# cunkai/index-tts-ipex

Hardware: AMD Instinct MI355X
Metric: audio_sec_per_sec (higher is better)
Workload: dtype bf16; 1 GPU; IndexTTS-1.5, 1 utterance(s)/GPU x 2 sentences x (L=105 text tokens, T=480 mel codes), prompt 511 frames, greedy fixed-length decode, rep_penalty 10; utterances_per_gpu=1, decode_batch=2

## Files before the change

### index-tts-ipex_amd/csrc/decode_engine.hip

```cpp
#include <cstdlib>
#include <type_traits>

#include "itts_decode.h"
#include "itts_engine_kernel.h"
#include "itts_sampler_dev.h"
#include "decode_pinned.h"

#ifndef ITTS_KV_PREFETCH
#define ITTS_KV_PREFETCH 1
#endif
#ifndef ITTS_EARLY_KV
#define ITTS_EARLY_KV 0
#endif

namespace itts {
namespace {

typedef unsigned int u32x4 __attribute__((ext_vector_type(4)));
typedef float f32x4 __attribute__((ext_vector_type(4)));
typedef uint32_t u32x2 __attribute__((ext_vector_type(2)));
typedef bf16_t bf16x2_t __attribute__((ext_vector_type(2)));
typedef unsigned long long u64;

template <int CTRL>
// ... 393 lines not shown
      for (int e = 0; e < 4; ++e) r2.xv[j][e] = ln_affine_rn(r2.xv[j][e], gm[j][e], bt[j][e]);
    ln_row_moments<K>(r2, 0.f, red + RED2 + grp2 * 8, tr);
  }
  __syncthreads();
  if (grp >= 0) {
    ln_row_norm<K>(r, 0.f, red + RED2 + grp * 8, eps);
    ln_row_store<K>(r, sxb + grp * (K / 2), tr);
  }
  if (NB > 4 && grp2 >= 0) {
    ln_row_norm<K>(r2, 0.f, red + RED2 + grp2 * 8, eps);
    ln_row_store<K>(r2, sxb + grp2 * (K / 2), tr);
  }
  __syncthreads();
}

template <int NB, bool ANC>
__global__ __launch_bounds__(1024) void decode_engine_kernel(EngArgs a) {
  constexpr int D = ENG_D, H = ENG_H, DH = 64, NCU = ENG_NCU;
  constexpr int GPH = NCU / H;
  constexpr int QO = 3 * DH / GPH;
  constexpr int HO = D / NCU;
  constexpr int FO = 4 * D / NCU;
  constexpr int NCW = 11;
  static_assert(GPH * QO == 3 * DH && HO * NCU == D && FO * NCU == 4 * D && (FO % 2) == 0, "partition");
  static_assert(QO <= 2 * NCW && HO <= NCW && FO / 2 <= NCW, "wave assignment");
  constexpr int NIT = 3, NSPLIT = 4, SLOTS = 32, LPK = 8, VEC = 8, UNC = 2;
  constexpr int SD = 2;
  static_assert(ATTN_NSPLIT == NSPLIT, "split count of the launch path");
  static_assert(NB <= ENG_MAX_ROWS, "LDS budget");

  extern __shared__ __attribute__((aligned(1024))) unsigned char smem[];
// ... 26 lines not shown
  const unsigned lds0 = (unsigned)(uintptr_t)(__attribute__((address_space(3))) unsigned char*)smem;
  const unsigned S0 = lds0, S1 = lds0 + SLOT, S2 = SLOT3 ? lds0 + 2 * SLOT : S1;
  static_assert(SLOT + SLOTB + (SLOT3 ? SLOTC : 0) + NB * D * 2 + NB * 4 * D * 2 + (SLOT3 ? NB * D * 4 + NB * D * 2 : 0) + (NB > 4 ? 512 : 256) +
                        (NB > 4 ? NB : 4) * 32 + (3 * DH + 16 * DH + 32 + NSPLIT * DH + 8 + 1) * 4 <= 160 * 1024, "LDS budget");
  const unsigned own_lds = lds0 + (unsigned)(reinterpret_cast<unsigned char*>(own) - smem);

  const int t = threadIdx.x, lane = t & 63;
  const int wave = __builtin_amdgcn_readfirstlane(t >> 6);
  const int cu = blockIdx.x;
  const bool gw = wave < 4;
  const bool lw = wave == 4;
  const bool cwv = wave > 4;
  const int cw = wave - 5;
  const int gh = cu / GPH, gm = cu % GPH;
  const bool qcu = cu < H * GPH;
  const bool acu = qcu && gm < NB;
  const int an0 = (gm / 4) * D + gh * DH + (gm % 4) * QO;

  Rt rt;
  rt.t0 = __builtin_amdgcn_s_memrealtime();
  const u64 clk0 = __builtin_amdgcn_s_memtime();
  rt.limit = a.timeout_ticks;
  rt.ctr = a.ctr;
  rt.dead = false;
  rt.first_delay = a.first_delay;
  rt.pass_sleep = a.pass_sleep;
  rt.tag = __builtin_amdgcn_readfirstlane(a.ctr[0]);
  const int prefix = __builtin_amdgcn_readfirstlane(a.prefix[0]);
  const int my_pos = acu ? __builtin_amdgcn_readfirstlane(prefix + a.len[acu ? gm : 0]) : 0;
  const int my_ks = acu ? __builtin_amdgcn_readfirstlane(a.kv_start[acu ? gm : 0]) : 0;
  const int my_par = (ANC && acu) ? __builtin_amdgcn_readfirstlane(a.len[acu ? gm : 0] & 1) : 0;

  if (t == 0) *own = 0;
  unsigned phase = 0;
  auto phase_done = [&](int ln_) {
    if (cwv && ln_ == 0) __hip_atomic_fetch_add(own, 1u, __ATOMIC_RELAXED, __HIP_MEMORY_SCOPE_WORKGROUP);
    ++phase;
  };
  if (lw) {
    if (SLOT3) dma_rows<HO, D>(a.L[0].wp, a.L[0].bp, cu * HO, S2, lane);
    if (qcu && HALFB) {
      dma_rows_at<QA1, D>(a.L[0].wa, an0, S0 + QOFF1, lane);
      dma_rows_at<QO - QA1, D>(a.L[0].wa, an0 + QA1, S0 + 256, lane);
      if (lane < QO) dma4(a.L[0].ba + an0 + lane, S0);
    } else if (qcu) {
      dma_rows<QO, D>(a.L[0].wa, a.L[0].ba, an0, S0, lane);
    }
  }
  if (t < NB * HO) hown[(t / HO) * 8 + t % HO] = a.h[(size_t)(t / HO) * D + cu * HO + t % HO];

  __builtin_amdgcn_s_waitcnt(0x0F70);
  constexpr size_t LSTRIDE = (size_t)NB * D * 15 / 2;
  constexpr size_t OQKV = 0, OCTX = (size_t)NB * 3 * D, OH1 = OCTX + NB * D / 2, OACT = OH1 + NB * D, OH2 = OACT + NB * 2 * D;
  for (int l = 0; l < a.NL; ++l) {
    const EngLayerW& w = a.L[l];
    int tl = t;
    asm volatile("" : "+v"(tl));
    const int ll = tl & 63;
    u64* __restrict__ G = a.gran + (size_t)l * LSTRIDE;

    constexpr int NIT_ = 3, NSPLIT_ = 4, SLOTS_ = 32, LPK_ = 8, VEC_ = 8, UNC_ = 2;
    KVec kr[2 * NIT_], vr[2 * NIT_];
    const int a_sp = wave >> 2, a_atid = (wave & 3) * 64 + ll, a_slot = a_atid / LPK_, a_sub = a_atid % LPK_;
    const size_t a_lo = ((size_t)l * a.B * H + (size_t)(acu ? gm : 0) * H + gh) * a.Smax * DH;
    const uint8_t* a_arow = nullptr;
    size_t a_lbase = 0;
    if constexpr (ANC) {
      a_arow = a.anc + ((size_t)my_par * a.B + (acu ? gm : 0)) * a.Smax;
      a_lbase = ((size_t)l * a.B + (size_t)((acu ? gm : 0) / a.nb) * a.nb) * H;
    }
    auto krow = [&](int j) -> const bf16_t* {
      if constexpr (ANC) return a.kc + ((a_lbase + (size_t)min((int)a_arow[j], a.nb - 1) * H + gh) * a.Smax + j) * DH;
      return a.kc + a_lo + (size_t)j * DH;
    };
    auto vrow = [&](int j) -> const bf16_t* {
      if constexpr (ANC) return a.vc + ((a_lbase + (size_t)min((int)a_arow[j], a.nb - 1) * H + gh) * a.Smax + j) * DH;
      return a.vc + a_lo + (size_t)j * DH;
    };
    auto kv_issue = [&](auto lo_c, auto hi_c) {
      constexpr int LO = decltype(lo_c)::value, HI = decltype(hi_c)::value;
#pragma unroll
      for (int u = LO; u < HI; ++u)
        if (u < UNC_ || (u * NSPLIT_ + a_sp) * SLOTS_ < my_pos + 1) {
          const int j = min((u * NSPLIT_ + a_sp) * SLOTS_ + a_slot, a.Smax - 1);
          kr[u].load(krow(j) + a_sub * VEC_);
          vr[u].load(vrow(j) + a_sub * VEC_);
        }
      __builtin_amdgcn_sched_barrier(0);
    };
    constexpr int EKV = ITTS_EARLY_KV;
    using Ic0 = std::integral_constant<int, 0>;
    using IcE = std::integral_constant<int, EKV>;
    using IcN = std::integral_constant<int, 2 * NIT_>;
    unsigned pf_sink = 0;
    if (ITTS_KV_PREFETCH && acu && cwv) {
      const int c0 = cw * 64 + ll;
      for (int j = my_ks + c0; j < my_pos; j += NCW * 64) {
        const char* pk = reinterpret_cast<const char*>(krow(j));
        const char* pv = reinterpret_cast<const char*>(vrow(j));
        asm volatile("global_load_dword %0, %1, off\n\tglobal_load_dword %0, %1, off offset:64\n\t"
                     "global_load_dword %0, %2, off\n\tglobal_load_dword %0, %2, off offset:64"
                     : "+v"(pf_sink)
                     : "v"(pk), "v"(pv)
                     : "memory");
      }
    }
    const bool early_kv = acu && EKV > 0;
    if (early_kv && cwv) kv_issue(Ic0{}, IcE{});

    if (gw) {
      if (l == 0) {
        for (int i = tl; i < NB * D; i += 256) xf[i] = a.h[i];
        __builtin_amdgcn_s_waitcnt(0x0F70);
      } else {
        wait_own(own_lds, NCW * phase, rt);
        sweep2<(NB * D / 2 + 255) / 256, false>(G - LSTRIDE + OH2, NB * D / 2 / a.fake_div, tl, rt, [&](int i, uint32_t v) { xf[i] = __uint_as_float(v); }, rt.first_delay);
      }
      if (early_kv) kv_issue(Ic0{}, IcE{});
    } else if (lw) {
      if (HALFB && l > 0 && qcu) {
        wait_own(own_lds, NCW * phase, rt);
        dma_rows_at<QO - QA1, D>(w.wa, an0 + QA1, S0 + 256, ll);
      }
      dma_wait_keep<0>();
      if (early_kv) kv_issue(Ic0{}, IcE{});
    }
    ENG_STAMP(0)
    __syncthreads();
    ENG_STAMP(1)
    ln_to_sxb<NB, D>(xf, xn, red, tl, a.eps);
    if (SLOT3) {
      if (lw && !acu) dma_rows<HO, 4 * D>(w.w2, w.b2, cu * HO, S1, ll);
    } else if (lw) {
      dma_rows<HO, D>(w.wp, w.bp, cu * HO, S1, ll);
    }
    if (qcu && cwv) {
#pragma unroll
      for (int s = 0; s < 2; ++s) {
        const int r = cw + NCW * s;
        if (r < QO) {
// ... 4 lines not shown
          float mine = 0.f;
#pragma unroll
          for (int b = 0; b < NB; ++b) {
            const float x = wave_sum_rl(acc[b]);
            mine = ll == b ? x : mine;
          }
          if (ll < NB) {
            st_gran(G + OQKV + (size_t)ll * 3 * D + an0 + r, rt.tag, __float_as_uint(mine + reinterpret_cast<const float*>(W0)[r]));
            if (a.dbg && l == a.dbg_layer) a.dbg[(size_t)ll * 3 * D + an0 + r] = mine + reinterpret_cast<const float*>(W0)[r];
          }
        }
      }
    }

    phase_done(ll);
    if (a.early_fc > 0 && lw && !acu) {
      wait_own(own_lds, NCW * phase, rt);
      for (int z = 0; z < a.early_fc; ++z) __builtin_amdgcn_s_sleep(1);
      dma_rows<FO, D>(w.wf, w.bf, cu * FO, S0, ll);
    }
    ENG_STAMP(8)

    if (acu) {
      const int sp = a_sp, atid = a_atid, slot = a_slot, sub = a_sub;
      bf16_t* kb = a.kc + a_lo;
      bf16_t* vb = a.vc + a_lo;
      kv_issue(IcE{}, IcN{});
      const int pos = my_pos, S = pos + 1, ks = my_ks;
      __builtin_amdgcn_sched_barrier(0);
      if (gw && tl < 3 * DH) {
        const u64* __restrict__ p = G + OQKV + (size_t)gm * 3 * D + (tl / DH) * D + gh * DH + tl % DH;
        wait_own(own_lds, NCW * phase, rt);
        unsigned spins = 0;
        while (!rt.dead) {
          const u64 x = ld_gran1(p);
          if ((unsigned)(x >> 32) == rt.tag) {
            qkvs[tl] = __uint_as_float((uint32_t)x);
            break;
          }
          if (spin_fail(rt, spins)) break;
          __builtin_amdgcn_s_sleep(1);
        }
      }
      ENG_STAMP(2)
      if (ITTS_KV_PREFETCH && cwv) asm volatile("s_waitcnt vmcnt(0)" : "+v"(pf_sink) : : "memory");
      __syncthreads();
      float qr[VEC];
      const bool own = atid < LPK && sp == 0;
#pragma unroll
      for (int i = 0; i < VEC; ++i) qr[i] = qkvs[sub * VEC + i] * a.scale;
      if (own) {
#pragma unroll
        for (int i = 0; i < VEC; ++i) {
          kb[(size_t)pos * DH + sub * VEC + i] = (bf16_t)qkvs[DH + sub * VEC + i];
          vb[(size_t)pos * DH + sub * VEC + i] = (bf16_t)qkvs[2 * DH + sub * VEC + i];
        }
      }
      float m = -INFINITY, lsum = 0.f, acc[VEC];
#pragma unroll
      for (int i = 0; i < VEC; ++i) acc[i] = 0.f;
      auto score = [&](const KVec& kk) {
        float sc = 0.f;
#pragma unroll
        for (int i = 0; i < VEC; ++i) sc = fmaf(qr[i], kk.get(i), sc);
        sc = dpp_add<0xB1>(sc);
        sc = dpp_add<0x4E>(sc);
        sc = dpp_add<0x141>(sc);
        return sc;
      };
      {
        float sc[2 * NIT + 1];
#pragma unroll
        for (int u = 0; u < 2 * NIT; ++u) {
          const int j = (u * NSPLIT + sp) * SLOTS + slot;
          sc[u] = -INFINITY;
          if (u < UNC || (u * NSPLIT + sp) * SLOTS < S) {
            const float tt = score(kr[u]);
            sc[u] = (j < S && j >= ks && j != pos) ? tt : -INFINITY;
          }
        }
        {
          float tt = 0.f;
#pragma unroll
          for (int i = 0; i < VEC; ++i) tt = fmaf(qr[i], own ? (float)(bf16_t)qkvs[DH + sub * VEC + i] : 0.f, tt);
          tt = dpp_add<0xB1>(tt);
          tt = dpp_add<0x4E>(tt);
          tt = dpp_add<0x141>(tt);
          sc[2 * NIT] = (slot == 0 && sp == 0) ? tt : -INFINITY;
        }
        float mw = sc[0];
#pragma unroll
        for (int u = 1; u <= 2 * NIT; ++u) mw = fmaxf(mw, sc[u]);
        if (mw > -INFINITY) {
#pragma unroll
          for (int u = 0; u < 2 * NIT; ++u)
            if (u < UNC || (u * NSPLIT + sp) * SLOTS < S) {
              const float p = __expf(sc[u] - mw);
              lsum += p;
#pragma unroll
              for (int i = 0; i < VEC; ++i) acc[i] = fmaf(p, vr[u].get(i), acc[i]);
            }
          const float p = __expf(sc[2 * NIT] - mw);
          lsum += p;
#pragma unroll
          for (int i = 0; i < VEC; ++i) acc[i] = fmaf(p, own ? (float)(bf16_t)qkvs[2 * DH + sub * VEC + i] : 0.f, acc[i]);
          m = mw;
        }
      }
      auto consume = [&](const KVec& kk, const KVec& vv, int j) {
        const bool ok = j < S && j >= ks && j != pos;
        float sc = score(kk);
        sc = ok ? sc : -INFINITY;
        const float mn = fmaxf(m, sc);
        const float corr = mn > -INFINITY ? __expf(m - mn) : 1.f;
        const float p = ok ? __expf(sc - mn) : 0.f;
        lsum = fmaf(lsum, corr, p);
#pragma unroll
        for (int i = 0; i < VEC; ++i) acc[i] = fmaf(p, ok ? vv.get(i) : 0.f, acc[i] * corr);
        m = mn;
      };
      for (int cb = 2 * NIT; (cb * NSPLIT + sp) * SLOTS < S; cb += SD) {
        KVec k2[SD], v2[SD];
#pragma unroll
        for (int u = 0; u < SD; ++u) {
          const int j = min(((cb + u) * NSPLIT + sp) * SLOTS + slot, a.Smax - 1);
          k2[u].load(krow(j) + sub * VEC);
          v2[u].load(vrow(j) + sub * VEC);
        }
#pragma unroll
        for (int u = 0; u < SD; ++u) consume(k2[u], v2[u], ((cb + u) * NSPLIT + sp) * SLOTS + slot);
      }
      auto bfly_max = [&](float x, int o) {
        if (o == 8) return fmaxf(x, __int_as_float(__builtin_amdgcn_update_dpp(0, __float_as_int(x), 0x128, 0xf, 0xf, true)));
        const u32x2 r = o == 16 ? __builtin_amdgcn_permlane16_swap(__float_as_uint(x), __float_as_uint(x), false, false)
                                : __builtin_amdgcn_permlane32_swap(__float_as_uint(x), __float_as_uint(x), false, false);
        return fmaxf(__uint_as_float(r[0]), __uint_as_float(r[1]));
      };
      auto bfly_sum = [&](float x, int o) {
        if (o == 8) return x + __int_as_float(__builtin_amdgcn_update_dpp(0, __float_as_int(x), 0x128, 0xf, 0xf, true));
        const u32x2 r = o == 16 ? __builtin_amdgcn_permlane16_swap(__float_as_uint(x), __float_as_uint(x), false, false)
                                : __builtin_amdgcn_permlane32_swap(__float_as_uint(x), __float_as_uint(x), false, false);
        return __uint_as_float(r[0]) + __uint_as_float(r[1]);
      };
      float M = m;
#pragma unroll
      for (int o = LPK; o < 64; o <<= 1) M = bfly_max(M, o);
      const float sc0 = M > -INFINITY ? __expf(m - M) : 0.f;
      lsum *= sc0;
#pragma unroll
      for (int i = 0; i < VEC; ++i) acc[i] *= sc0;
#pragma unroll
      for (int o = LPK; o < 64; o <<= 1) {
        lsum = bfly_sum(lsum, o);
#pragma unroll
        for (int i = 0; i < VEC; ++i) acc[i] = bfly_sum(acc[i], o);
      }
      if (ll < LPK)
#pragma unroll
        for (int i = 0; i < VEC; ++i) so[wave * DH + ll * VEC + i] = acc[i];
      if (ll == 0) {
        smx[wave] = M;
        slx[wave] = lsum;
      }
      __syncthreads();
      if (atid < DH) {
        float MM = smx[4 * sp];
#pragma unroll
        for (int i = 1; i < 4; ++i) MM = fmaxf(MM, smx[4 * sp + i]);
        float o = 0.f, L = 0.f;
#pragma unroll
        for (int i = 0; i < 4; ++i) {
          const float e = smx[4 * sp + i] > -INFINITY ? __expf(smx[4 * sp + i] - MM) : 0.f;
          o = fmaf(e, so[(4 * sp + i) * DH + atid], o);
          L = fmaf(e, slx[4 * sp + i], L);
        }
        po[sp * DH + atid] = o;
        if (atid == 0) {
          pml[sp] = MM;
          pml[NSPLIT + sp] = L;
        }
      }
      __syncthreads();
      if (tl < DH / 2) {
        const float Mx = fmaxf(fmaxf(pml[0], pml[1]), fmaxf(pml[2], pml[3]));
        float wgt[NSPLIT], L = 0.f;
#pragma unroll
        for (int s2 = 0; s2 < NSPLIT; ++s2) {
          wgt[s2] = pml[s2] > -INFINITY ? __expf(pml[s2] - Mx) : 0.f;
          L = fmaf(wgt[s2], pml[NSPLIT + s2], L);
        }
        const float inv = 1.f / L;
        float xm[2];
#pragma unroll
        for (int e = 0; e < 2; ++e) {
          float v = 0.f;
#pragma unroll
          for (int s2 = 0; s2 < NSPLIT; ++s2) v = fmaf(wgt[s2], po[s2 * DH + 2 * tl + e], v);
          xm[e] = v * inv;
        }
        st_gran(G + OCTX + (size_t)gm * (D / 2) + gh * (DH / 2) + tl, rt.tag, pack_bf16(xm[0], xm[1]));
      }
      ENG_STAMP(3)
    }

    if (gw) {
      if (acu)
        sweep2<(NB * D / 4 + 255) / 256, false>(G + OCTX, NB * D / 4, tl, rt, [&](int i, uint32_t v) { xc[i] = v; }, rt.first_delay);
      else
        sweep2<(NB * D / 4 + 255) / 256, true>(G + OCTX, NB * D / 4, tl, rt, [&](int i, uint32_t v) { xc[i] = v; }, a.ctx_delay);
    } else if (!SLOT3 && lw) {
      dma_wait_keep<0>();
    }
    ENG_STAMP(4)
    __syncthreads();
    if (lw && !(a.early_fc > 0 && !acu)) {
      if (a.thin_fc)
        dma_rows<FO, D, 12>(w.wf, w.bf, cu * FO, S0, ll);
      else
        dma_rows<FO, D>(w.wf, w.bf, cu * FO, S0, ll);
    }
    if (cwv && cw < HO) {
      float acc[NB];
#pragma unroll
      for (int b = 0; b < NB; ++b) acc[b] = 0.f;
      dots<NB, D>(W2 + 256 + cw * D * 2, xc, ll, acc);
      float mine = 0.f;
#pragma unroll
      for (int b = 0; b < NB; ++b) {
        const float x = wave_sum_rl(acc[b]);
        mine = ll == b ? x : mine;
// ... 288 lines not shown
    }
  }
  if (cu == 0 && t == 0) a.ctr[0] = rt.tag + 1 == 0 ? 1u : rt.tag + 1;
  if (a.stamp && t == 0) {
    const u64 c1 = __builtin_amdgcn_s_memtime(), r1 = __builtin_amdgcn_s_memrealtime();
    a.stamp[(size_t)cu * a.NL * 16 + 15] = (unsigned)((c1 - clk0) * 1000 / (r1 - rt.t0 + 1));
    if (a.NL >= 3) {
      a.stamp[((size_t)cu * a.NL + 1) * 16 + 15] = (unsigned)rt.t0;
      a.stamp[((size_t)cu * a.NL + 2) * 16 + 15] = (unsigned)r1;
    }
  }
}

}

size_t eng_gran_count(int layers) { return (size_t)layers * ENG_MAX_ROWS * ENG_D * 15 / 2 + ENG_CAND_WORDS; }

int decode_engine_layers(const EngArgs& a, hipStream_t s) {
  ITTS_REQUIRE(a.B >= 1 && a.B <= ENG_MAX_ROWS && a.NL >= 1 && a.NL <= ENG_MAX_LAYERS && a.gran && a.h && a.kc && a.vc && a.ctr, "decode_engine: bad arguments");
  const size_t lds = 160 * 1024;
#define ITTS_ENG_GO(NB, ANC_)                                                                                                   \
  {                                                                                                                             \
    static bool attr = false;                                                                                                   \
    if (!attr) {                                                                                                                \
      ITTS_HIP_CHECK(hipFuncSetAttribute(reinterpret_cast<const void*>(&decode_engine_kernel<NB, ANC_>),                        \
                                         hipFuncAttributeMaxDynamicSharedMemorySize, (int)lds));                                \
      attr = true;                                                                                                              \
    }                                                                                                                           \
    hipLaunchKernelGGL((decode_engine_kernel<NB, ANC_>), dim3(ENG_NCU), dim3(1024), lds, s, a);                                 \
  }
  if (a.anc) {
    ITTS_REQUIRE(a.nb >= 2 && a.nb <= a.B && a.B % a.nb == 0, "decode_engine: beam ancestry needs B to be a multiple of 2 <= nb <= B");
    if (a.B == 2) ITTS_ENG_GO(2, true)
    else if (a.B == 3) ITTS_ENG_GO(3, true)
    else if (a.B == 4) ITTS_ENG_GO(4, true)
    else if (a.B == 5) ITTS_ENG_GO(5, true)
    else ITTS_ENG_GO(6, true)
  } else if (a.B == 1) ITTS_ENG_GO(1, false)
  else if (a.B == 2) ITTS_ENG_GO(2, false)
  else if (a.B == 3) ITTS_ENG_GO(3, false)
  else if (a.B == 4) ITTS_ENG_GO(4, false)
  else if (a.B == 5) ITTS_ENG_GO(5, false)
  else ITTS_ENG_GO(6, false)
#undef ITTS_ENG_GO
  ITTS_HIP_CHECK(hipGetLastError());
  return OK;
}

}
```

### index-tts-ipex_amd/csrc/engine.h

```cpp
#pragma once
#include <map>
#include <utility>
#include <string>
#include <unordered_map>
#include <vector>

#include "../../include/itts_hip.h"
#include "itts_decode.h"
#include "itts_engine_kernel.h"
#include "itts_kernels.h"

namespace itts {

struct Tensor {
  const void* p = nullptr;
  int dt = 0, nd = 0;
  int64_t d[4] = {0, 0, 0, 0};
  int64_t numel() const {
    int64_t n = 1;
    for (int i = 0; i < nd; ++i) n *= d[i];
    return n;
  }
};

// ... 115 lines not shown
  int *cand_tok = nullptr, *cand_n = nullptr;
  int *hyp_tok = nullptr, *hyp_len = nullptr, *hyp_order = nullptr, *hyp_n = nullptr, *hyp_counter = nullptr, *beam_done = nullptr;
  float *hyp_score = nullptr, *hyp_worst = nullptr;
  size_t beam_cap = 0;
  int beam_rows = 0, beam_gen = 0, beam_smax = 0;
  unsigned long long* gran = nullptr;
  int* fuse_err = nullptr;
  int fuse_failed = 0;
  int fuse = 0, graph_fuse = 0;
  unsigned long long* eng_gran = nullptr;
  unsigned* eng_ctr = nullptr;
  int eng_off = 0;
  int eng_force = 0;
  int eng_failed = 0;
  int graph_eng = 0;
  int graph_mode = 0;
  float typical_mass = 0.f, graph_typical = 0.f;
  float* scores2 = nullptr;
  int* forced = nullptr;
  int use_forced = 0, graph_forced = 0;
  int host_sample = 0, graph_host_sample = 0;
  int input_n = 0, graph_input_n = 0;
  int last_mode = 0;
  float graph_penalty = 0.f;
  bool active = false;
};

struct Engine {
  itts_config cfg;
  int adt = 0;
// ... 81 lines not shown
  std::vector<int32_t> forced_host;
  int forced_B = 0, forced_n = 0;
  int gpt_status(int* steps, int* n_unf, hipStream_t s);
  int gpt_fetch(int32_t* codes, float* logits, hipStream_t s);
  int gpt_latent(const float* cond, const int32_t* text_ids, int L, const int32_t* codes, int T, void* latent_out,
                 hipStream_t s);
  int gpt_latent_batch(const float* cond, const int32_t* text_ids, const int* Ls, const int32_t* codes, const int* Ts,
                       int nseq, void* latent_out, hipStream_t s);
  int bigvgan(const void* latent, const float* spk, int B, int T, float* wav, hipStream_t s);
  int dvae_decode(const int32_t* codes, int B, int T, void* mel_out, hipStream_t s);
  int dvae_encode(const void* mel, int B, int T, int32_t* codes_host, hipStream_t s);

  int gpt_layers_full(float* h, int B, int S, const int* kv_start_dev, bool write_cache, hipStream_t s);
  int decode_step_launch(hipStream_t s);
  bool engine_usable() const;
  int ensure_engine_state(hipStream_t s);
  int engine_check(hipStream_t s);
  int head_and_sample(hipStream_t s, bool have_logits = false, bool sampled = false);
  int sample_from_logits(hipStream_t s, bool sampled = false);
  SamplerArgs greedy_sampler_args(const float* lg_in, bool typical) const;
  int ensure_decode_state(int B, int Smax, int max_gen, hipStream_t s);
  template <typename F>
  int two_pass(F&& body, hipStream_t s) {
    dry = true;
    ws_reset();
    int st = body();
    dry = false;
    if (st != OK) return st;
    ITTS_TRY(ws_reserve(ws_off + 4096, s));
    ws_reset();
// ... 6 lines not shown
```

### index-tts-ipex_amd/csrc/itts_engine_kernel.h

```cpp
#pragma once
#include "itts_common.h"
#include "itts_decode.h"

namespace itts {

constexpr int ENG_D = 1280, ENG_H = 20, ENG_NCU = 256, ENG_MAX_ROWS = 6;
constexpr int ENG_MAX_LAYERS = 24;
constexpr bool ENG_DEFAULT_ON = true;

struct EngLayerW {
  const bf16_t *wa, *wp, *wf, *w2;
  const float *ba, *bp, *bf, *b2;
};

struct EngArgs {
  EngLayerW L[ENG_MAX_LAYERS];
  unsigned long long* gran = nullptr;
  float* h = nullptr;
  bf16_t* kc = nullptr;
  bf16_t* vc = nullptr;
  const int* len = nullptr;
  const int* kv_start = nullptr;
  const int* prefix = nullptr;
  unsigned* ctr = nullptr;
// ... 2 lines not shown
  int NL = 0, B = 0, Smax = 0;
  float scale = 0.125f, eps = 1e-5f;
  unsigned timeout_ticks = 2000000;
  int first_delay = 14, pass_sleep = 1;
  int ctx_delay = 0, act_delay = 16;
  const bf16_t* head_w = nullptr;
  const float* head_b = nullptr;
  const float* lnf_g = nullptr;
  const float* lnf_b = nullptr;
  float* logits = nullptr;
  int V = 0;
  int fold_sampler = 0;
  SamplerArgs samp;
  unsigned long long* cand = nullptr;
  int early_fc = 0;
  int early_kv = 1;
  int fake_div = 1;
  int thin_fc = 0;
  float* dbg = nullptr;
  int dbg_layer = -1;
  unsigned* stamp = nullptr;
};

size_t eng_gran_count(int layers);
constexpr size_t ENG_CAND_WORDS = (size_t)ENG_MAX_ROWS * ENG_NCU * 2;
int decode_engine_layers(const EngArgs& a, hipStream_t s);

}
```

### index-tts-ipex_amd/csrc/model_gpt.hip

```cpp
#include <algorithm>
#include <atomic>
#include <cstdio>
#include <cmath>
#include <cstring>
#include <mutex>

#include <cstdlib>

#include "engine.h"

namespace itts {

namespace {

struct RowDesc {
  int kind, a, b, pad;
};

template <typename TW>
__global__ void gpt_embed_rows_kernel(float* __restrict__ h, const RowDesc* __restrict__ rd, const float* __restrict__ cond,
                                      const TW* __restrict__ text_emb, const TW* __restrict__ text_pos,
                                      const TW* __restrict__ mel_emb, const TW* __restrict__ mel_pos, int D) {
  const int r = blockIdx.x;
  const RowDesc d = rd[r];
// ... 132 lines not shown
  if (hipGetDevice(&dev) != hipSuccess) return false;
  int ncu = ncu_of[dev & 63].load(std::memory_order_relaxed);
  if (ncu == 0) {
    if (hipDeviceGetAttribute(&ncu, hipDeviceAttributeMultiprocessorCount, dev) != hipSuccess || ncu <= 0) ncu = -1;
    ncu_of[dev & 63].store(ncu, std::memory_order_relaxed);
  }
  const itts_config& c = cfg;
  if ((env_off && !ds.eng_force) || ds.eng_off || ds.eng_failed || ncu != ENG_NCU) return false;
  if (ds.fuse && !ds.fuse_failed) return false;
  if (adt != BF16 || ds.B < 1 || ds.B > ENG_MAX_ROWS || ds.nb < 1 || ds.B % ds.nb != 0 || (ds.nb > 1 && !ds.anc)) return false;
  if (c.model_dim != ENG_D || c.heads != ENG_H || c.layers < 1 || c.layers > ENG_MAX_LAYERS || ds.Smax > 2048 || ds.Smax % 256 != 0) return false;
  for (const GptLayerW& L : gpt.layers)
    for (const Lin* l : {&L.attn, &L.proj, &L.fc, &L.proj2})
      if (l->dt != BF16 || l->w8 || !l->b || l->taps != 1) return false;
  return true;
}

int Engine::ensure_engine_state(hipStream_t s) {
  DecodeState& d = ds;
  if (d.eng_gran) return OK;
  const itts_config& c = cfg;
  for (int l = 0; l < c.layers; ++l) {
    const GptLayerW& L = gpt.layers[l];
    ITTS_REQUIRE(L.attn.N == 3 * ENG_D && L.attn.Cin == ENG_D && L.proj.N == ENG_D && L.proj.Cin == ENG_D &&
                     L.fc.N == 4 * ENG_D && L.fc.Cin == ENG_D && L.proj2.N == ENG_D && L.proj2.Cin == 4 * ENG_D,
                 "decode engine: projection shapes");
  }
  const size_t gb = eng_gran_count(c.layers) * 8;
  ITTS_TRY(dev_alloc((void**)&d.eng_gran, gb));
  ITTS_TRY(dev_alloc((void**)&d.eng_ctr, 64));
// ... 527 lines not shown
    ea.scale = 1.f / std::sqrt((float)dh);
    static const int e_tap = getenv("ITTS_TAP_LAYER") ? atoi(getenv("ITTS_TAP_LAYER")) : -1;
    if (debug && e_tap >= 0 && e_tap < eng_first && !dry) {
      ea.dbg = ds.act;
      ea.dbg_layer = e_tap;
    }
    static const int e_fd_env = getenv("ITTS_ENGINE_FIRST_DELAY") ? atoi(getenv("ITTS_ENGINE_FIRST_DELAY")) : -1;
    static const int e_ad_env = getenv("ITTS_ENGINE_ACT_DELAY") ? atoi(getenv("ITTS_ENGINE_ACT_DELAY")) : -1;
    const int e_fd = e_fd_env >= 0 ? e_fd_env : (B <= 2 ? 14 : 12);
    const int e_ad = e_ad_env >= 0 ? e_ad_env : (B <= 2 ? 16 : B <= 4 ? 8 : 4);
    static const int e_ps = getenv("ITTS_ENGINE_PASS_SLEEP") ? atoi(getenv("ITTS_ENGINE_PASS_SLEEP")) : 1;
    static const int e_thin = getenv("ITTS_ENGINE_THIN_FC") ? atoi(getenv("ITTS_ENGINE_THIN_FC")) : 0;
    ea.thin_fc = e_thin;
    static const int e_early = getenv("ITTS_ENGINE_EARLY_FC") ? atoi(getenv("ITTS_ENGINE_EARLY_FC")) : -1;
    ea.early_fc = e_early >= 0 ? e_early : 74;
    ea.first_delay = e_fd;
    static const int e_fake = getenv("ITTS_ENG_FAKE_DIV") ? atoi(getenv("ITTS_ENG_FAKE_DIV")) : 1;
    ea.fake_div = e_fake < 1 ? 1 : e_fake;
    static const int e_ekv = getenv("ITTS_ENGINE_EARLY_KV") ? atoi(getenv("ITTS_ENGINE_EARLY_KV")) : 1;
    ea.early_kv = e_ekv;
    static const int e_cd = getenv("ITTS_ENGINE_CTX_DELAY") ? atoi(getenv("ITTS_ENGINE_CTX_DELAY")) : 0;
    ea.ctx_delay = e_cd;
    ea.act_delay = e_ad;
    ea.pass_sleep = e_ps;
    if (const char* tt = getenv("ITTS_ENGINE_TIMEOUT_TICKS")) ea.timeout_ticks = (unsigned)atol(tt);
    static const bool e_stamps = getenv("ITTS_ENGINE_STAMPS") != nullptr;
    if (debug && e_stamps && !dry) ea.stamp = (unsigned*)ds.scores2;
    ds.last_mode = eng_first > 0;
    static const bool e_head = !(getenv("ITTS_ENGINE_HEAD") && atoi(getenv("ITTS_ENGINE_HEAD")) == 0);
    const bool fold_head = e_head && eng_first == c.layers && gpt.head.dt == BF16 && !gpt.head.w8 && gpt.head.b && gpt.head.Cin == ENG_D &&
// ... 337 lines not shown
  ITTS_HIP_CHECK(hipGetDevice(&dev));
  EngineGate& g = engine_gate(dev);
  std::lock_guard<std::mutex> lk(g.mu);
  if (!g.ev) ITTS_HIP_CHECK(hipEventCreateWithFlags(&g.ev, hipEventDisableTiming));
  else ITTS_HIP_CHECK(hipStreamWaitEvent(s, g.ev, 0));
  const int rc = gpt_decode_steps(nsteps, s);
  ITTS_HIP_CHECK(hipEventRecord(g.ev, s));
  return rc;
}

int Engine::gpt_decode_steps(int nsteps, hipStream_t s) {
  ITTS_REQUIRE(nsteps >= 0, "gpt_decode: nsteps < 0");
  if (use_graph && s != nullptr) {
    DecodeState& d = ds;
    const bool stale = !d.graph || d.graph_B != d.B || d.graph_Smax != d.Smax || d.graph_max_gen != d.max_gen ||
                       d.graph_forced != d.use_forced || d.graph_input_n != d.input_n || d.graph_host_sample != d.host_sample || d.graph_fuse != (d.fuse && !d.fuse_failed) || d.graph_eng != (int)engine_usable() || d.graph_nb != d.nb || d.graph_beam_sample != d.beam_sample ||
                       d.graph_length_penalty != d.length_penalty || d.graph_typical != d.typical_mass || d.graph_penalty != d.penalty || d.graph_suppress != d.suppress_stop || d.graph_sample != d.do_sample ||
                       d.graph_top_k != d.top_k || d.graph_top_p != d.top_p || d.graph_temperature != d.temperature;
    static const int GK = [] {
      const char* e = getenv("ITTS_GRAPH_STEPS");
      const int v = e ? atoi(e) : 8;
      return v < 1 ? 1 : (v > 32 ? 32 : v);
    }();
    if (stale && nsteps > 0) {
      for (hipGraphExec_t* ge : {&d.graph, &d.graphK})
        if (*ge) {
          (void)hipGraphExecDestroy(*ge);
          *ge = nullptr;
        }
      for (int which = 0; which < (GK > 1 ? 2 : 1); ++which) {
        hipGraph_t g = nullptr;
// ... 5 lines not shown
          if (g) (void)hipGraphDestroy(g);
          return st;
        }
        ITTS_HIP_CHECK(ee);
        ITTS_HIP_CHECK(hipGraphInstantiate(which ? &d.graphK : &d.graph, g, nullptr, nullptr, 0));
        (void)hipGraphDestroy(g);
      }
      d.graph_B = d.B;
      d.graph_Smax = d.Smax;
      d.graph_max_gen = d.max_gen;
      d.graph_forced = d.use_forced;
      d.graph_input_n = d.input_n;
      d.graph_host_sample = d.host_sample;
      d.graph_fuse = d.fuse && !d.fuse_failed;
      d.graph_eng = (int)engine_usable();
      d.graph_mode = d.last_mode;
      d.graph_nb = d.nb;
      d.graph_beam_sample = d.beam_sample;
      d.graph_length_penalty = d.length_penalty;
      d.graph_typical = d.typical_mass;
      d.graph_penalty = d.penalty;
      d.graph_suppress = d.suppress_stop;
      d.graph_sample = d.do_sample;
      d.graph_top_k = d.top_k;
      d.graph_top_p = d.top_p;
      d.graph_temperature = d.temperature;
    }
    d.last_mode = d.graph_mode;
    int left = nsteps;
    if (d.graphK)
// ... 160 lines not shown
```

Measured before the change: 179.5 audio-s/s.

## Spread per-row decode attention splits across four workgroups with global partial merge

For small decode batches (up to 3 rows), each row's attention over the KV cache is split across four workgroups of the head group instead of four wave groups within one workgroup. The non-zero splits write partial max/sum/output to a new global partials region and the split-0 workgroup merges them. This spreads KV-cache reads across more CUs and adjusts the prefetch and early-FC scheduling to match. The cost is an extra cross-workgroup handoff through global memory and more complex synchronisation. Attention waves in spread mode are limited to waves 12 and up.

New measurement: 171.6 audio-s/s (median of 2 runs). 0.956x the previous value.

```diff
diff --git a/index-tts-ipex_amd/csrc/decode_engine.hip b/index-tts-ipex_amd/csrc/decode_engine.hip
--- a/index-tts-ipex_amd/csrc/decode_engine.hip
+++ b/index-tts-ipex_amd/csrc/decode_engine.hip
@@ -431,7 +431,7 @@
   __syncthreads();
 }
 
-template <int NB, bool ANC>
+template <int NB, bool ANC, bool SPREAD>
 __global__ __launch_bounds__(1024) void decode_engine_kernel(EngArgs a) {
   constexpr int D = ENG_D, H = ENG_H, DH = 64, NCU = ENG_NCU;
   constexpr int GPH = NCU / H;
@@ -488,7 +488,14 @@
   const int cw = wave - 5;
   const int gh = cu / GPH, gm = cu % GPH;
   const bool qcu = cu < H * GPH;
-  const bool acu = qcu && gm < NB;
+  constexpr bool spread = SPREAD;
+  static_assert(!SPREAD || (NB <= ENG_SPREAD_ROWS && 4 * NB <= GPH), "split workgroups of a head group");
+  const bool acu = qcu && gm < (spread ? 4 * NB : NB);
+  const int arow = spread ? gm % NB : gm;
+  const int asp = spread ? gm / NB : 0;
+  const bool amerge = acu && asp == 0;
+  const bool lacu = acu && !spread;
+  const bool aw = !spread || wave >= 12;
   const int an0 = (gm / 4) * D + gh * DH + (gm % 4) * QO;
 
   Rt rt;
@@ -501,9 +508,9 @@
   rt.pass_sleep = a.pass_sleep;
   rt.tag = __builtin_amdgcn_readfirstlane(a.ctr[0]);
   const int prefix = __builtin_amdgcn_readfirstlane(a.prefix[0]);
-  const int my_pos = acu ? __builtin_amdgcn_readfirstlane(prefix + a.len[acu ? gm : 0]) : 0;
-  const int my_ks = acu ? __builtin_amdgcn_readfirstlane(a.kv_start[acu ? gm : 0]) : 0;
-  const int my_par = (ANC && acu) ? __builtin_amdgcn_readfirstlane(a.len[acu ? gm : 0] & 1) : 0;
+  const int my_pos = acu ? __builtin_amdgcn_readfirstlane(prefix + a.len[acu ? arow : 0]) : 0;
+  const int my_ks = acu ? __builtin_amdgcn_readfirstlane(a.kv_start[acu ? arow : 0]) : 0;
+  const int my_par = (ANC && acu) ? __builtin_amdgcn_readfirstlane(a.len[acu ? arow : 0] & 1) : 0;
 
   if (t == 0) *own = 0;
   unsigned phase = 0;
@@ -525,6 +532,7 @@
 
   __builtin_amdgcn_s_waitcnt(0x0F70);
   constexpr size_t LSTRIDE = (size_t)NB * D * 15 / 2;
+  constexpr size_t PSTRIDE = SPREAD ? (size_t)NB * H * 3 * 66 : 0;
   constexpr size_t OQKV = 0, OCTX = (size_t)NB * 3 * D, OH1 = OCTX + NB * D / 2, OACT = OH1 + NB * D, OH2 = OACT + NB * 2 * D;
   for (int l = 0; l < a.NL; ++l) {
     const EngLayerW& w = a.L[l];
@@ -532,16 +540,17 @@
     asm volatile("" : "+v"(tl));
     const int ll = tl & 63;
     u64* __restrict__ G = a.gran + (size_t)l * LSTRIDE;
+    u64* __restrict__ P = a.part + (size_t)l * PSTRIDE;
 
     constexpr int NIT_ = 3, NSPLIT_ = 4, SLOTS_ = 32, LPK_ = 8, VEC_ = 8, UNC_ = 2;
     KVec kr[2 * NIT_], vr[2 * NIT_];
-    const int a_sp = wave >> 2, a_atid = (wave & 3) * 64 + ll, a_slot = a_atid / LPK_, a_sub = a_atid % LPK_;
-    const size_t a_lo = ((size_t)l * a.B * H + (size_t)(acu ? gm : 0) * H + gh) * a.Smax * DH;
+    const int a_sp = spread ? asp : wave >> 2, a_atid = (wave & 3) * 64 + ll, a_slot = a_atid / LPK_, a_sub = a_atid % LPK_;
+    const size_t a_lo = ((size_t)l * a.B * H + (size_t)(acu ? arow : 0) * H + gh) * a.Smax * DH;
     const uint8_t* a_arow = nullptr;
     size_t a_lbase = 0;
     if constexpr (ANC) {
-      a_arow = a.anc + ((size_t)my_par * a.B + (acu ? gm : 0)) * a.Smax;
-      a_lbase = ((size_t)l * a.B + (size_t)((acu ? gm : 0) / a.nb) * a.nb) * H;
+      a_arow = a.anc + ((size_t)my_par * a.B + (acu ? arow : 0)) * a.Smax;
+      a_lbase = ((size_t)l * a.B + (size_t)((acu ? arow : 0) / a.nb) * a.nb) * H;
     }
     auto krow = [&](int j) -> const bf16_t* {
       if constexpr (ANC) return a.kc + ((a_lbase + (size_t)min((int)a_arow[j], a.nb - 1) * H + gh) * a.Smax + j) * DH;
@@ -569,7 +578,10 @@
     unsigned pf_sink = 0;
     if (ITTS_KV_PREFETCH && acu && cwv) {
       const int c0 = cw * 64 + ll;
-      for (int j = my_ks + c0; j < my_pos; j += NCW * 64) {
+      for (int i = c0;; i += NCW * 64) {
+        const int j = spread ? ((i / SLOTS_) * NSPLIT_ + a_sp) * SLOTS_ + i % SLOTS_ : my_ks + i;
+        if (j >= my_pos) break;
+        if (j < my_ks) continue;
         const char* pk = reinterpret_cast<const char*>(krow(j));
         const char* pv = reinterpret_cast<const char*>(vrow(j));
         asm volatile("global_load_dword %0, %1, off\n\tglobal_load_dword %0, %1, off offset:64\n\t"
@@ -579,7 +591,7 @@
                      : "memory");
       }
     }
-    const bool early_kv = acu && EKV > 0;
+    const bool early_kv = acu && !spread && EKV > 0;
     if (early_kv && cwv) kv_issue(Ic0{}, IcE{});
 
     if (gw) {
@@ -598,6 +610,8 @@
       }
       dma_wait_keep<0>();
       if (early_kv) kv_issue(Ic0{}, IcE{});
+    } else if (ITTS_KV_PREFETCH && acu) {
+      asm volatile("s_waitcnt vmcnt(0)" : "+v"(pf_sink) : : "memory");
     }
     ENG_STAMP(0)
     __syncthreads();
@@ -632,7 +646,8 @@
     }
 
     phase_done(ll);
-    if (a.early_fc > 0 && lw && !acu) {
+    const bool fc_early = a.early_fc > 0 && (!acu || (!lacu && a.early_fc_attn));
+    if (fc_early && lw) {
       wait_own(own_lds, NCW * phase, rt);
       for (int z = 0; z < a.early_fc; ++z) __builtin_amdgcn_s_sleep(1);
       dma_rows<FO, D>(w.wf, w.bf, cu * FO, S0, ll);
@@ -643,11 +658,11 @@
       const int sp = a_sp, atid = a_atid, slot = a_slot, sub = a_sub;
       bf16_t* kb = a.kc + a_lo;
       bf16_t* vb = a.vc + a_lo;
-      kv_issue(IcE{}, IcN{});
+      if (!spread) kv_issue(IcE{}, IcN{});
       const int pos = my_pos, S = pos + 1, ks = my_ks;
       __builtin_amdgcn_sched_barrier(0);
       if (gw && tl < 3 * DH) {
-        const u64* __restrict__ p = G + OQKV + (size_t)gm * 3 * D + (tl / DH) * D + gh * DH + tl % DH;
+        const u64* __restrict__ p = G + OQKV + (size_t)arow * 3 * D + (tl / DH) * D + gh * DH + tl % DH;
         wait_own(own_lds, NCW * phase, rt);
         unsigned spins = 0;
         while (!rt.dead) {
@@ -661,127 +676,130 @@
         }
       }
       ENG_STAMP(2)
-      if (ITTS_KV_PREFETCH && cwv) asm volatile("s_waitcnt vmcnt(0)" : "+v"(pf_sink) : : "memory");
       __syncthreads();
-      float qr[VEC];
-      const bool own = atid < LPK && sp == 0;
-#pragma unroll
-      for (int i = 0; i < VEC; ++i) qr[i] = qkvs[sub * VEC + i] * a.scale;
-      if (own) {
-#pragma unroll
-        for (int i = 0; i < VEC; ++i) {
-          kb[(size_t)pos * DH + sub * VEC + i] = (bf16_t)qkvs[DH + sub * VEC + i];
-          vb[(size_t)pos * DH + sub * VEC + i] = (bf16_t)qkvs[2 * DH + sub * VEC + i];
-        }
-      }
-      float m = -INFINITY, lsum = 0.f, acc[VEC];
-#pragma unroll
-      for (int i = 0; i < VEC; ++i) acc[i] = 0.f;
-      auto score = [&](const KVec& kk) {
-        float sc = 0.f;
-#pragma unroll
-        for (int i = 0; i < VEC; ++i) sc = fmaf(qr[i], kk.get(i), sc);
-        sc = dpp_add<0xB1>(sc);
-        sc = dpp_add<0x4E>(sc);
-        sc = dpp_add<0x141>(sc);
-        return sc;
-      };
-      {
-        float sc[2 * NIT + 1];
-#pragma unroll
-        for (int u = 0; u < 2 * NIT; ++u) {
-          const int j = (u * NSPLIT + sp) * SLOTS + slot;
-          sc[u] = -INFINITY;
-          if (u < UNC || (u * NSPLIT + sp) * SLOTS < S) {
-            const float tt = score(kr[u]);
-            sc[u] = (j < S && j >= ks && j != pos) ? tt : -INFINITY;
-          }
-        }
+      if (aw) {
+        if (spread) kv_issue(Ic0{}, IcN{});
+        float qr[VEC];
+        const bool own = atid < LPK && sp == 0;
+#pragma unroll
+        for (int i = 0; i < VEC; ++i) qr[i] = qkvs[sub * VEC + i] * a.scale;
+        if (own) {
+#pragma unroll
+          for (int i = 0; i < VEC; ++i) {
+            kb[(size_t)pos * DH + sub * VEC + i] = (bf16_t)qkvs[DH + sub * VEC + i];
+            vb[(size_t)pos * DH + sub * VEC + i] = (bf16_t)qkvs[2 * DH + sub * VEC + i];
+          }
+        }
+        float m = -INFINITY, lsum = 0.f, acc[VEC];
+#pragma unroll
+        for (int i = 0; i < VEC; ++i) acc[i] = 0.f;
+        auto score = [&](const KVec& kk) {
+          float sc = 0.f;
+#pragma unroll
+          for (int i = 0; i < VEC; ++i) sc = fmaf(qr[i], kk.get(i), sc);
+          sc = dpp_add<0xB1>(sc);
+          sc = dpp_add<0x4E>(sc);
+          sc = dpp_add<0x141>(sc);
+          return sc;
+        };
         {
-          float tt = 0.f;
-#pragma unroll
-          for (int i = 0; i < VEC; ++i) tt = fmaf(qr[i], own ? (float)(bf16_t)qkvs[DH + sub * VEC + i] : 0.f, tt);
-          tt = dpp_add<0xB1>(tt);
-          tt = dpp_add<0x4E>(tt);
-          tt = dpp_add<0x141>(tt);
-          sc[2 * NIT] = (slot == 0 && sp == 0) ? tt : -INFINITY;
-        }
-        float mw = sc[0];
-#pragma unroll
-        for (int u = 1; u <= 2 * NIT; ++u) mw = fmaxf(mw, sc[u]);
-        if (mw > -INFINITY) {
-#pragma unroll
-          for (int u = 0; u < 2 * NIT; ++u)
+          float sc[2 * NIT + 1];
+#pragma unroll
+          for (int u = 0; u < 2 * NIT; ++u) {
+            const int j = (u * NSPLIT + sp) * SLOTS + slot;
+            sc[u] = -INFINITY;
             if (u < UNC || (u * NSPLIT + sp) * SLOTS < S) {
-              const float p = __expf(sc[u] - mw);
-              lsum += p;
-#pragma unroll
-              for (int i = 0; i < VEC; ++i) acc[i] = fmaf(p, vr[u].get(i), acc[i]);
+              const float tt = score(kr[u]);
+              sc[u] = (j < S && j >= ks && j != pos) ? tt : -INFINITY;
             }
-          const float p = __expf(sc[2 * NIT] - mw);
-          lsum += p;
-#pragma unroll
-          for (int i = 0; i < VEC; ++i) acc[i] = fmaf(p, own ? (float)(bf16_t)qkvs[2 * DH + sub * VEC + i] : 0.f, acc[i]);
-          m = mw;
-        }
-      }
-      auto consume = [&](const KVec& kk, const KVec& vv, int j) {
-        const bool ok = j < S && j >= ks && j != pos;
-        float sc = score(kk);
-        sc = ok ? sc : -INFINITY;
-        const float mn = fmaxf(m, sc);
-        const float corr = mn > -INFINITY ? __expf(m - mn) : 1.f;
-        const float p = ok ? __expf(sc - mn) : 0.f;
-        lsum = fmaf(lsum, corr, p);
-#pragma unroll
-        for (int i = 0; i < VEC; ++i) acc[i] = fmaf(p, ok ? vv.get(i) : 0.f, acc[i] * corr);
-        m = mn;
-      };
-      for (int cb = 2 * NIT; (cb * NSPLIT + sp) * SLOTS < S; cb += SD) {
-        KVec k2[SD], v2[SD];
-#pragma unroll
-        for (int u = 0; u < SD; ++u) {
-          const int j = min(((cb + u) * NSPLIT + sp) * SLOTS + slot, a.Smax - 1);
-          k2[u].load(krow(j) + sub * VEC);
-          v2[u].load(vrow(j) + sub * VEC);
-        }
-#pragma unroll
-        for (int u = 0; u < SD; ++u) consume(k2[u], v2[u], ((cb + u) * NSPLIT + sp) * SLOTS + slot);
-      }
-      auto bfly_max = [&](float x, int o) {
-        if (o == 8) return fmaxf(x, __int_as_float(__builtin_amdgcn_update_dpp(0, __float_as_int(x), 0x128, 0xf, 0xf, true)));
-        const u32x2 r = o == 16 ? __builtin_amdgcn_permlane16_swap(__float_as_uint(x), __float_as_uint(x), false, false)
-                                : __builtin_amdgcn_permlane32_swap(__float_as_uint(x), __float_as_uint(x), false, false);
-        return fmaxf(__uint_as_float(r[0]), __uint_as_float(r[1]));
-      };
-      auto bfly_sum = [&](float x, int o) {
-        if (o == 8) return x + __int_as_float(__builtin_amdgcn_update_dpp(0, __float_as_int(x), 0x128, 0xf, 0xf, true));
-        const u32x2 r = o == 16 ? __builtin_amdgcn_permlane16_swap(__float_as_uint(x), __float_as_uint(x), false, false)
-                                : __builtin_amdgcn_permlane32_swap(__float_as_uint(x), __float_as_uint(x), false, false);
-        return __uint_as_float(r[0]) + __uint_as_float(r[1]);
-      };
-      float M = m;
-#pragma unroll
-      for (int o = LPK; o < 64; o <<= 1) M = bfly_max(M, o);
-      const float sc0 = M > -INFINITY ? __expf(m - M) : 0.f;
-      lsum *= sc0;
-#pragma unroll
-      for (int i = 0; i < VEC; ++i) acc[i] *= sc0;
-#pragma unroll
-      for (int o = LPK; o < 64; o <<= 1) {
-        lsum = bfly_sum(lsum, o);
-#pragma unroll
-        for (int i = 0; i < VEC; ++i) acc[i] = bfly_sum(acc[i], o);
-      }
-      if (ll < LPK)
-#pragma unroll
-        for (int i = 0; i < VEC; ++i) so[wave * DH + ll * VEC + i] = acc[i];
-      if (ll == 0) {
-        smx[wave] = M;
-        slx[wave] = lsum;
+          }
+          {
+            float tt = 0.f;
+#pragma unroll
+            for (int i = 0; i < VEC; ++i) tt = fmaf(qr[i], own ? (float)(bf16_t)qkvs[DH + sub * VEC + i] : 0.f, tt);
+            tt = dpp_add<0xB1>(tt);
+            tt = dpp_add<0x4E>(tt);
+            tt = dpp_add<0x141>(tt);
+            sc[2 * NIT] = (slot == 0 && sp == 0) ? tt : -INFINITY;
+          }
+          float mw = sc[0];
+#pragma unroll
+          for (int u = 1; u <= 2 * NIT; ++u) mw = fmaxf(mw, sc[u]);
+          if (mw > -INFINITY) {
+#pragma unroll
+            for (int u = 0; u < 2 * NIT; ++u)
+              if (u < UNC || (u * NSPLIT + sp) * SLOTS < S) {
+                const float p = __expf(sc[u] - mw);
+                lsum += p;
+#pragma unroll
+                for (int i = 0; i < VEC; ++i) acc[i] = fmaf(p, vr[u].get(i), acc[i]);
+              }
+            const float p = __expf(sc[2 * NIT] - mw);
+            lsum += p;
+#pragma unroll
+            for (int i = 0; i < VEC; ++i) acc[i] = fmaf(p, own ? (float)(bf16_t)qkvs[2 * DH + sub * VEC + i] : 0.f, acc[i]);
+            m = mw;
+          }
+        }
+        auto consume = [&](const KVec& kk, const KVec& vv, int j) {
+          const bool ok = j < S && j >= ks && j != pos;
+          float sc = score(kk);
+          sc = ok ? sc : -INFINITY;
+          const float mn = fmaxf(m, sc);
+          const float corr = mn > -INFINITY ? __expf(m - mn) : 1.f;
+          const float p = ok ? __expf(sc - mn) : 0.f;
+          lsum = fmaf(lsum, corr, p);
+#pragma unroll
+          for (int i = 0; i < VEC; ++i) acc[i] = fmaf(p, ok ? vv.get(i) : 0.f, acc[i] * corr);
+          m = mn;
+        };
+        for (int cb = 2 * NIT; (cb * NSPLIT + sp) * SLOTS < S; cb += SD) {
+          KVec k2[SD], v2[SD];
+#pragma unroll
+          for (int u = 0; u < SD; ++u) {
+            const int j = min(((cb + u) * NSPLIT + sp) * SLOTS + slot, a.Smax - 1);
+            k2[u].load(krow(j) + sub * VEC);
+            v2[u].load(vrow(j) + sub * VEC);
+          }
+#pragma unroll
+          for (int u = 0; u < SD; ++u) consume(k2[u], v2[u], ((cb + u) * NSPLIT + sp) * SLOTS + slot);
+        }
+        auto bfly_max = [&](float x, int o) {
+          if (o == 8) return fmaxf(x, __int_as_float(__builtin_amdgcn_update_dpp(0, __float_as_int(x), 0x128, 0xf, 0xf, true)));
+          const u32x2 r = o == 16 ? __builtin_amdgcn_permlane16_swap(__float_as_uint(x), __float_as_uint(x), false, false)
+                                  : __builtin_amdgcn_permlane32_swap(__float_as_uint(x), __float_as_uint(x), false, false);
+          return fmaxf(__uint_as_float(r[0]), __uint_as_float(r[1]));
+        };
+        auto bfly_sum = [&](float x, int o) {
+          if (o == 8) return x + __int_as_float(__builtin_amdgcn_update_dpp(0, __float_as_int(x), 0x128, 0xf, 0xf, true));
+          const u32x2 r = o == 16 ? __builtin_amdgcn_permlane16_swap(__float_as_uint(x), __float_as_uint(x), false, false)
+                                  : __builtin_amdgcn_permlane32_swap(__float_as_uint(x), __float_as_uint(x), false, false);
+          return __uint_as_float(r[0]) + __uint_as_float(r[1]);
+        };
+        float M = m;
+#pragma unroll
+        for (int o = LPK; o < 64; o <<= 1) M = bfly_max(M, o);
+        const float sc0 = M > -INFINITY ? __expf(m - M) : 0.f;
+        lsum *= sc0;
+#pragma unroll
+        for (int i = 0; i < VEC; ++i) acc[i] *= sc0;
+#pragma unroll
+        for (int o = LPK; o < 64; o <<= 1) {
+          lsum = bfly_sum(lsum, o);
+#pragma unroll
+          for (int i = 0; i < VEC; ++i) acc[i] = bfly_sum(acc[i], o);
+        }
+        const int sw = 4 * sp + (wave & 3);
+        if (ll < LPK)
+#pragma unroll
+          for (int i = 0; i < VEC; ++i) so[sw * DH + ll * VEC + i] = acc[i];
+        if (ll == 0) {
+          smx[sw] = M;
+          slx[sw] = lsum;
+        }
       }
       __syncthreads();
-      if (atid < DH) {
+      if (aw && atid < DH) {
         float MM = smx[4 * sp];
 #pragma unroll
         for (int i = 1; i < 4; ++i) MM = fmaxf(MM, smx[4 * sp + i]);
@@ -792,37 +810,65 @@
           o = fmaf(e, so[(4 * sp + i) * DH + atid], o);
           L = fmaf(e, slx[4 * sp + i], L);
         }
-        po[sp * DH + atid] = o;
-        if (atid == 0) {
-          pml[sp] = MM;
-          pml[NSPLIT + sp] = L;
-        }
-      }
-      __syncthreads();
-      if (tl < DH / 2) {
-        const float Mx = fmaxf(fmaxf(pml[0], pml[1]), fmaxf(pml[2], pml[3]));
-        float wgt[NSPLIT], L = 0.f;
-#pragma unroll
-        for (int s2 = 0; s2 < NSPLIT; ++s2) {
-          wgt[s2] = pml[s2] > -INFINITY ? __expf(pml[s2] - Mx) : 0.f;
-          L = fmaf(wgt[s2], pml[NSPLIT + s2], L);
-        }
-        const float inv = 1.f / L;
-        float xm[2];
-#pragma unroll
-        for (int e = 0; e < 2; ++e) {
-          float v = 0.f;
-#pragma unroll
-          for (int s2 = 0; s2 < NSPLIT; ++s2) v = fmaf(wgt[s2], po[s2 * DH + 2 * tl + e], v);
-          xm[e] = v * inv;
-        }
-        st_gran(G + OCTX + (size_t)gm * (D / 2) + gh * (DH / 2) + tl, rt.tag, pack_bf16(xm[0], xm[1]));
-      }
-      ENG_STAMP(3)
+        if (spread && sp != 0) {
+          u64* __restrict__ pp = P + ((size_t)(arow * H + gh) * 3 + (sp - 1)) * 66;
+          st_gran(pp + atid, rt.tag, __float_as_uint(o));
+          if (atid == 0) {
+            st_gran(pp + DH, rt.tag, __float_as_uint(MM));
+            st_gran(pp + DH + 1, rt.tag, __float_as_uint(L));
+            if (a.stamp) a.stamp[((size_t)cu * a.NL + l) * 16 + 3] = (unsigned)__builtin_amdgcn_s_memrealtime();
+          }
+        } else {
+          po[sp * DH + atid] = o;
+          if (atid == 0) {
+            pml[sp] = MM;
+            pml[NSPLIT + sp] = L;
+          }
+        }
+      }
+      if (spread && amerge && gw && tl < 3 * 66) {
+        const int s1 = 1 + tl / 66, k = tl % 66;
+        const u64* __restrict__ p = P + (size_t)(arow * H + gh) * 3 * 66 + tl;
+        unsigned spins = 0;
+        while (!rt.dead) {
+          const u64 x = ld_gran1(p);
+          if ((unsigned)(x >> 32) == rt.tag) {
+            const float v = __uint_as_float((uint32_t)x);
+            if (k < DH) po[s1 * DH + k] = v;
+            else pml[(k - DH) * NSPLIT + s1] = v;
+            break;
+          }
+          if (spin_fail(rt, spins)) break;
+          __builtin_amdgcn_s_sleep(1);
+        }
+      }
+      if (amerge) {
+        __syncthreads();
+        if (tl < DH / 2) {
+          const float Mx = fmaxf(fmaxf(pml[0], pml[1]), fmaxf(pml[2], pml[3]));
+          float wgt[NSPLIT], L = 0.f;
+#pragma unroll
+          for (int s2 = 0; s2 < NSPLIT; ++s2) {
+            wgt[s2] = pml[s2] > -INFINITY ? __expf(pml[s2] - Mx) : 0.f;
+            L = fmaf(wgt[s2], pml[NSPLIT + s2], L);
+          }
+          const float inv = 1.f / L;
+          float xm[2];
+#pragma unroll
+          for (int e = 0; e < 2; ++e) {
+            float v = 0.f;
+#pragma unroll
+            for (int s2 = 0; s2 < NSPLIT; ++s2) v = fmaf(wgt[s2], po[s2 * DH + 2 * tl + e], v);
+            xm[e] = v * inv;
+          }
+          st_gran(G + OCTX + (size_t)arow * (D / 2) + gh * (DH / 2) + tl, rt.tag, pack_bf16(xm[0], xm[1]));
+        }
+        ENG_STAMP(3)
+      }
     }
 
     if (gw) {
-      if (acu)
+      if (amerge)
         sweep2<(NB * D / 4 + 255) / 256, false>(G + OCTX, NB * D / 4, tl, rt, [&](int i, uint32_t v) { xc[i] = v; }, rt.first_delay);
       else
         sweep2<(NB * D / 4 + 255) / 256, true>(G + OCTX, NB * D / 4, tl, rt, [&](int i, uint32_t v) { xc[i] = v; }, a.ctx_delay);
@@ -831,7 +877,7 @@
     }
     ENG_STAMP(4)
     __syncthreads();
-    if (lw && !(a.early_fc > 0 && !acu)) {
+    if (lw && !fc_early) {
       if (a.thin_fc)
         dma_rows<FO, D, 12>(w.wf, w.bf, cu * FO, S0, ll);
       else
@@ -1150,20 +1196,26 @@
 
 }
 
-size_t eng_gran_count(int layers) { return (size_t)layers * ENG_MAX_ROWS * ENG_D * 15 / 2 + ENG_CAND_WORDS; }
+size_t eng_gran_count(int layers) { return eng_part_offset(layers) + (size_t)layers * ENG_PART_WORDS + ENG_CAND_WORDS; }
 
 int decode_engine_layers(const EngArgs& a, hipStream_t s) {
   ITTS_REQUIRE(a.B >= 1 && a.B <= ENG_MAX_ROWS && a.NL >= 1 && a.NL <= ENG_MAX_LAYERS && a.gran && a.h && a.kc && a.vc && a.ctr, "decode_engine: bad arguments");
+  ITTS_REQUIRE(!a.attn_spread || (a.B <= ENG_SPREAD_ROWS && a.part), "decode_engine: the spread attention needs <= 3 rows and the partials region");
   const size_t lds = 160 * 1024;
-#define ITTS_ENG_GO(NB, ANC_)                                                                                                   \
+#define ITTS_ENG_GO1(NB, ANC_, SP_)                                                                                             \
   {                                                                                                                             \
     static bool attr = false;                                                                                                   \
     if (!attr) {                                                                                                                \
-      ITTS_HIP_CHECK(hipFuncSetAttribute(reinterpret_cast<const void*>(&decode_engine_kernel<NB, ANC_>),                        \
+      ITTS_HIP_CHECK(hipFuncSetAttribute(reinterpret_cast<const void*>(&decode_engine_kernel<NB, ANC_, SP_>),                   \
                                          hipFuncAttributeMaxDynamicSharedMemorySize, (int)lds));                                \
       attr = true;                                                                                                              \
     }                                                                                                                           \
-    hipLaunchKernelGGL((decode_engine_kernel<NB, ANC_>), dim3(ENG_NCU), dim3(1024), lds, s, a);                                 \
+    hipLaunchKernelGGL((decode_engine_kernel<NB, ANC_, SP_>), dim3(ENG_NCU), dim3(1024), lds, s, a);                            \
+  }
+#define ITTS_ENG_GO(NB, ANC_)                                                                                                   \
+  {                                                                                                                             \
+    if (a.attn_spread) ITTS_ENG_GO1(NB, ANC_, (NB <= ENG_SPREAD_ROWS))                                                          \
+    else ITTS_ENG_GO1(NB, ANC_, false)                                                                                          \
   }
   if (a.anc) {
     ITTS_REQUIRE(a.nb >= 2 && a.nb <= a.B && a.B % a.nb == 0, "decode_engine: beam ancestry needs B to be a multiple of 2 <= nb <= B");
@@ -1179,6 +1231,7 @@
   else if (a.B == 5) ITTS_ENG_GO(5, false)
   else ITTS_ENG_GO(6, false)
 #undef ITTS_ENG_GO
+#undef ITTS_ENG_GO1
   ITTS_HIP_CHECK(hipGetLastError());
   return OK;
 }
diff --git a/index-tts-ipex_amd/csrc/engine.h b/index-tts-ipex_amd/csrc/engine.h
--- a/index-tts-ipex_amd/csrc/engine.h
+++ b/index-tts-ipex_amd/csrc/engine.h
@@ -153,6 +153,7 @@
   int eng_force = 0;
   int eng_failed = 0;
   int graph_eng = 0;
+  int graph_spread = 0;
   int graph_mode = 0;
   float typical_mass = 0.f, graph_typical = 0.f;
   float* scores2 = nullptr;
@@ -264,6 +265,7 @@
   int gpt_layers_full(float* h, int B, int S, const int* kv_start_dev, bool write_cache, hipStream_t s);
   int decode_step_launch(hipStream_t s);
   bool engine_usable() const;
+  bool engine_attn_spread() const;
   int ensure_engine_state(hipStream_t s);
   int engine_check(hipStream_t s);
   int head_and_sample(hipStream_t s, bool have_logits = false, bool sampled = false);
diff --git a/index-tts-ipex_amd/csrc/itts_engine_kernel.h b/index-tts-ipex_amd/csrc/itts_engine_kernel.h
--- a/index-tts-ipex_amd/csrc/itts_engine_kernel.h
+++ b/index-tts-ipex_amd/csrc/itts_engine_kernel.h
@@ -40,16 +40,22 @@
   SamplerArgs samp;
   unsigned long long* cand = nullptr;
   int early_fc = 0;
+  int early_fc_attn = 0;
   int early_kv = 1;
   int fake_div = 1;
   int thin_fc = 0;
   float* dbg = nullptr;
   int dbg_layer = -1;
+  int attn_spread = 0;
+  unsigned long long* part = nullptr;
   unsigned* stamp = nullptr;
 };
 
 size_t eng_gran_count(int layers);
 constexpr size_t ENG_CAND_WORDS = (size_t)ENG_MAX_ROWS * ENG_NCU * 2;
+constexpr int ENG_SPREAD_ROWS = 3;
+constexpr size_t ENG_PART_WORDS = (size_t)ENG_SPREAD_ROWS * ENG_H * 3 * 66;
+inline size_t eng_part_offset(int layers) { return (size_t)layers * ENG_MAX_ROWS * ENG_D * 15 / 2; }
 int decode_engine_layers(const EngArgs& a, hipStream_t s);
 
 }
diff --git a/index-tts-ipex_amd/csrc/model_gpt.hip b/index-tts-ipex_amd/csrc/model_gpt.hip
--- a/index-tts-ipex_amd/csrc/model_gpt.hip
+++ b/index-tts-ipex_amd/csrc/model_gpt.hip
@@ -170,6 +170,11 @@
     for (const Lin* l : {&L.attn, &L.proj, &L.fc, &L.proj2})
       if (l->dt != BF16 || l->w8 || !l->b || l->taps != 1) return false;
   return true;
+}
+
+bool Engine::engine_attn_spread() const {
+  const char* ev = getenv("ITTS_ENG_ATTN_SPREAD");
+  return ds.B <= ENG_SPREAD_ROWS && !(ev && atoi(ev) == 0);
 }
 
 int Engine::ensure_engine_state(hipStream_t s) {
@@ -727,6 +732,12 @@
     ea.thin_fc = e_thin;
     static const int e_early = getenv("ITTS_ENGINE_EARLY_FC") ? atoi(getenv("ITTS_ENGINE_EARLY_FC")) : -1;
     ea.early_fc = e_early >= 0 ? e_early : 74;
+    static const int e_early_attn = getenv("ITTS_ENGINE_EARLY_FC_ATTN") ? atoi(getenv("ITTS_ENGINE_EARLY_FC_ATTN")) : 0;
+    ea.early_fc_attn = e_early_attn;
+    if (engine_attn_spread()) {
+      ea.attn_spread = 1;
+      ea.part = ds.eng_gran + eng_part_offset(c.layers);
+    }
     ea.first_delay = e_fd;
     static const int e_fake = getenv("ITTS_ENG_FAKE_DIV") ? atoi(getenv("ITTS_ENG_FAKE_DIV")) : 1;
     ea.fake_div = e_fake < 1 ? 1 : e_fake;
@@ -1094,7 +1105,7 @@
   if (use_graph && s != nullptr) {
     DecodeState& d = ds;
     const bool stale = !d.graph || d.graph_B != d.B || d.graph_Smax != d.Smax || d.graph_max_gen != d.max_gen ||
-                       d.graph_forced != d.use_forced || d.graph_input_n != d.input_n || d.graph_host_sample != d.host_sample || d.graph_fuse != (d.fuse && !d.fuse_failed) || d.graph_eng != (int)engine_usable() || d.graph_nb != d.nb || d.graph_beam_sample != d.beam_sample ||
+                       d.graph_forced != d.use_forced || d.graph_input_n != d.input_n || d.graph_host_sample != d.host_sample || d.graph_fuse != (d.fuse && !d.fuse_failed) || d.graph_eng != (int)engine_usable() || d.graph_spread != (int)engine_attn_spread() || d.graph_nb != d.nb || d.graph_beam_sample != d.beam_sample ||
                        d.graph_length_penalty != d.length_penalty || d.graph_typical != d.typical_mass || d.graph_penalty != d.penalty || d.graph_suppress != d.suppress_stop || d.graph_sample != d.do_sample ||
                        d.graph_top_k != d.top_k || d.graph_top_p != d.top_p || d.graph_temperature != d.temperature;
     static const int GK = [] {
@@ -1130,6 +1141,7 @@
       d.graph_host_sample = d.host_sample;
       d.graph_fuse = d.fuse && !d.fuse_failed;
       d.graph_eng = (int)engine_usable();
+      d.graph_spread = (int)engine_attn_spread();
       d.graph_mode = d.last_mode;
       d.graph_nb = d.nb;
       d.graph_beam_sample = d.beam_sample;
```
